# marl/l3embedding

Measured on AMD Instinct MI355X. Metric: AVC training pairs/sec (1s audio + 224x224 frame), higher is better.
Workload: dtype f32; 1 GPU; full cnn_L3_melspec2 AVC training step (audio+vision+fusion, fwd+bwd+Adam), batch 64 per GPU, global batch 64, fp32, inputs resident in HBM; global_batch=64, parallelism=dp1, fp32_conv=f4x4

## Files before the change

include/l3hip.h:

```cpp
#ifndef L3HIP_H
#define L3HIP_H

#include <stdint.h>

#ifdef __cplusplus
extern "C" {
#endif

#define L3_OK 0
#define L3_EINVAL (-1)
#define L3_EHIP (-2)
#define L3_ENOMEM (-3)
#define L3_ESTATE (-4)
#define L3_ECOMM (-5)

#define L3_MODEL_CNN_L3_ORIG 0
#define L3_MODEL_TINY_L3 1
#define L3_MODEL_CNN_L3_KAPREDBINPUTBN 2
#define L3_MODEL_CNN_L3_MELSPEC1 3
#define L3_MODEL_CNN_L3_MELSPEC2 4

typedef struct l3_engine l3_engine;

#define L3_DTYPE_F32 0
// ... 82 lines not shown
int l3_comm_timing(l3_engine *e, int on);
int l3_comm_timing_read(l3_engine *e, double *exposed_ms, double *span_ms, double *bucket_ms, int cap, int *steps);

int l3_grad_arena_dev(l3_engine *e, void **dev_ptr, int64_t *numel);
int l3_bucket_range(const l3_engine *e, int bucket, int64_t *offset, int64_t *numel);
int l3_bn_stats_pack_dev(l3_engine *e, void **send_dev, int64_t *numel);
int l3_bn_stats_replicas_dev(l3_engine *e, int world, void **gathered_dev);

int l3_embed_audio(l3_engine *e, const float *audio, int64_t n, int pool_h, int pool_w, float *out);
int l3_embed_vision(l3_engine *e, const float *video, int64_t n, int pool_h, int pool_w, float *out);
int64_t l3_embed_dim(const l3_engine *e, int vision, int pool_h, int pool_w);
int l3_embed_audio_frames(l3_engine *e, const float *samples, int64_t n_samples, const int64_t *table,
                          int64_t n_frames, int pool_h, int pool_w, float *out);
int l3_embed_audio_clips_resampled(l3_engine *e, const float *native, int64_t n_native, const int64_t *clips,
                                   int64_t n_clips, const double *half_window, int64_t n_window, int num_table,
                                   int64_t n_samples, const int64_t *table, int64_t n_frames, int pool_h, int pool_w,
                                   float *out);

int l3_get_activation(l3_engine *e, const char *name, float *dst, int64_t numel);
int l3_activation_numel(l3_engine *e, const char *name, int64_t *numel);
int l3_sync(l3_engine *e);
int l3_profile_enable(l3_engine *e, int on);
int l3_set_tower_overlap(l3_engine *e, int on);
int l3_profile_read(l3_engine *e, int family, double *ms, int64_t *launches, double *flops);
int l3_profile_read_executed(l3_engine *e, int family, double *flops);
int l3_profile_read_bytes(l3_engine *e, int family, double *bytes);

#define L3_OP_BF16_STORED 2
#define L3_OP_BF16_STORED_OUT 3
int l3_op_conv2d_fwd_dt(int device, int dtype, const float *x, const float *w, const float *b, float *y,
                        int n, int h, int wd, int cin, int cout, int kh, int kw, int same);
int l3_op_conv2d_bwd_dt(int device, int dtype, const float *x, const float *w, const float *dy, float *dx,
                        float *dw, float *db, int n, int h, int wd, int cin, int cout, int kh, int kw, int same);
int l3_op_conv2d_fwd(int device, const float *x, const float *w, const float *b, float *y,
                     int n, int h, int wd, int cin, int cout, int kh, int kw, int same);
int l3_op_conv2d_bwd(int device, const float *x, const float *w, const float *dy,
                     float *dx, float *dw, float *db,
                     int n, int h, int wd, int cin, int cout, int kh, int kw, int same);
int l3_op_bn_relu_fwd(int device, const float *x, const float *gamma, const float *beta,
                      float *y, float *mean, float *var, int64_t rows, int c, int relu, int x_bf16);
int l3_op_bn_relu_bwd(int device, const float *x, const float *y, const float *dy,
                      const float *gamma, const float *beta, const float *mean, const float *var,
                      float *dx, float *dgamma, float *dbeta, int64_t rows, int c, int relu, int x_bf16);
int l3_op_bn_relu_pool2_fwd(int device, const float *x, const float *gamma, const float *beta, float *p,
                            float *mean, float *var, int n, int h, int wd, int c, int same, int relu_mode, int x_bf16);
int l3_op_bn_relu_pool2_bwd(int device, const float *x, const float *gamma, const float *beta, const float *dp,
                            float *dx, float *dgamma, float *dbeta, float *dbias, int n, int h, int wd, int c,
                            int same, int relu_mode, int x_bf16);
int l3_op_maxpool_fwd(int device, const float *x, float *y, int n, int h, int wd, int c,
                      int ph, int pw, int sh, int sw, int same);
int l3_op_maxpool_bwd(int device, const float *x, const float *dy, float *dx, int n, int h,
                      int wd, int c, int ph, int pw, int sh, int sw, int same);
int l3_op_frontend(int device, int model_type, const float *audio, int n, int db_max_scope, float *out);
int l3_op_gather_frames(int device, const float *samples, int64_t n_samples, const int64_t *table,
                        int64_t n_frames, float *frames);
int l3_op_resample(int device, const float *x, int64_t n_in, int64_t sr_orig, int64_t sr_new, const double *half_window,
                   int64_t n_window, int num_table, int64_t t0, int64_t n_out, float *y);
int l3_op_resample_clips(int device, const float *x, int64_t n_in, const int64_t *clips, int64_t n_clips, int64_t sr_new,
                         const double *half_window, int64_t n_window, int num_table, int64_t n_samples, int copy_equal,
                         float *y);
int l3_op_bn_stats_from_partials(int device, const float *part, int nblk, int c, const float *pivot, int64_t rows,
                                 float eps, float *mean, float *var);
int l3_op_preprocess(int device, const uint8_t *video_u8, int64_t nv, float *video,
                     const int16_t *audio_i16, int64_t na, float *audio);
int l3_op_augment_video(int device, const uint8_t *u8, int n, int h, int w, const l3_augment_params *params,
                        uint8_t *out_u8, float *out_f32);
// ... 124 lines not shown
```

l3embedding_amd/_lib.py:

```python
import ctypes as C
import os

import numpy as np

from . import _build

MODEL_IDS = {
    'cnn_L3_orig': 0,
    'tiny_L3': 1,
    'cnn_L3_kapredbinputbn': 2,
    'cnn_L3_melspec1': 3,
    'cnn_L3_melspec2': 4,
}

FAMILIES = ('conv_fwd', 'conv_dgrad', 'conv_wgrad', 'elementwise', 'frontend', 'head', 'adam')


DTYPES = {'f32': 0, 'fp32': 0, 'float32': 0, 'bf16': 1}
FP32_CONV = {'f4x4': 0, 'f2x2': 1, 'f2x2_bf16x6': 2}
DP_MOVING = {'replicas': 0, 'rank_local': 1}
OP_DTYPES = dict(DTYPES, bf16_stored=2, bf16_stored_out=3)


class L3Config(C.Structure):
# ... 60 lines not shown
    'l3_step_results_enqueue': (C.c_int, [C.c_void_p, C.c_int, C.c_int]),
    'l3_step_results_wait': (C.c_int, [C.c_void_p, C.c_int, C.POINTER(C.c_float), C.POINTER(C.c_float)]),
    'l3_comm_unique_id': (C.c_int, [C.c_void_p]),
    'l3_comm_init': (C.c_int, [C.c_void_p, C.c_void_p, C.c_int, C.c_int]),
    'l3_comm_destroy': (C.c_int, [C.c_void_p]),
    'l3_comm_info': (C.c_int, [C.c_void_p, C.POINTER(C.c_int), C.POINTER(C.c_int), C.c_char_p, C.c_int]),
    'l3_comm_allreduce_host': (C.c_int, [C.c_void_p, C.POINTER(C.c_double), C.c_int, C.c_int]),
    'l3_step_dp': (C.c_int, [C.c_void_p, C.c_float]),
    'l3_comm_timing': (C.c_int, [C.c_void_p, C.c_int]),
    'l3_comm_timing_read': (C.c_int, [C.c_void_p, C.POINTER(C.c_double), C.POINTER(C.c_double), C.POINTER(C.c_double), C.c_int, C.POINTER(C.c_int)]),
    'l3_grad_arena_dev': (C.c_int, [C.c_void_p, C.POINTER(C.c_void_p), C.POINTER(C.c_int64)]),
    'l3_bucket_range': (C.c_int, [C.c_void_p, C.c_int, C.POINTER(C.c_int64), C.POINTER(C.c_int64)]),
    'l3_embed_audio': (C.c_int, [C.c_void_p, C.c_void_p, C.c_int64, C.c_int, C.c_int, C.c_void_p]),
    'l3_embed_vision': (C.c_int, [C.c_void_p, C.c_void_p, C.c_int64, C.c_int, C.c_int, C.c_void_p]),
    'l3_embed_dim': (C.c_int64, [C.c_void_p, C.c_int, C.c_int, C.c_int]),
    'l3_embed_audio_frames': (C.c_int, [C.c_void_p, C.c_void_p, C.c_int64, C.c_void_p, C.c_int64, C.c_int, C.c_int,
                                        C.c_void_p]),
    'l3_embed_audio_clips_resampled': (C.c_int, [C.c_void_p, C.c_void_p, C.c_int64, C.c_void_p, C.c_int64, C.c_void_p,
                                                 C.c_int64, C.c_int, C.c_int64, C.c_void_p, C.c_int64, C.c_int, C.c_int,
                                                 C.c_void_p]),
    'l3_get_activation': (C.c_int, [C.c_void_p, C.c_char_p, C.c_void_p, C.c_int64]),
    'l3_activation_numel': (C.c_int, [C.c_void_p, C.c_char_p, C.POINTER(C.c_int64)]),
    'l3_sync': (C.c_int, [C.c_void_p]),
    'l3_profile_enable': (C.c_int, [C.c_void_p, C.c_int]),
    'l3_set_tower_overlap': (C.c_int, [C.c_void_p, C.c_int]),
    'l3_profile_read_executed': (C.c_int, [C.c_void_p, C.c_int, C.POINTER(C.c_double)]),
    'l3_profile_read_bytes': (C.c_int, [C.c_void_p, C.c_int, C.POINTER(C.c_double)]),
    'l3_profile_read': (C.c_int, [C.c_void_p, C.c_int, C.POINTER(C.c_double), C.POINTER(C.c_int64),
                                  C.POINTER(C.c_double)]),
    'l3_op_conv2d_fwd': (C.c_int, [C.c_int, C.c_void_p, C.c_void_p, C.c_void_p, C.c_void_p] + [C.c_int] * 8),
    'l3_op_conv2d_fwd_dt': (C.c_int, [C.c_int, C.c_int, C.c_void_p, C.c_void_p, C.c_void_p, C.c_void_p] + [C.c_int] * 8),
    'l3_op_conv2d_bwd_dt': (C.c_int, [C.c_int, C.c_int] + [C.c_void_p] * 6 + [C.c_int] * 8),
    'l3_op_conv2d_bwd': (C.c_int, [C.c_int] + [C.c_void_p] * 6 + [C.c_int] * 8),
    'l3_op_bn_relu_fwd': (C.c_int, [C.c_int] + [C.c_void_p] * 6 + [C.c_int64, C.c_int, C.c_int, C.c_int]),
    'l3_op_bn_relu_bwd': (C.c_int, [C.c_int] + [C.c_void_p] * 10 + [C.c_int64, C.c_int, C.c_int, C.c_int]),
    'l3_op_bn_relu_pool2_fwd': (C.c_int, [C.c_int] + [C.c_void_p] * 6 + [C.c_int] * 7),
    'l3_op_bn_relu_pool2_bwd': (C.c_int, [C.c_int] + [C.c_void_p] * 8 + [C.c_int] * 7),
    'l3_op_maxpool_fwd': (C.c_int, [C.c_int, C.c_void_p, C.c_void_p] + [C.c_int] * 9),
    'l3_op_maxpool_bwd': (C.c_int, [C.c_int, C.c_void_p, C.c_void_p, C.c_void_p] + [C.c_int] * 9),
    'l3_op_frontend': (C.c_int, [C.c_int, C.c_int, C.c_void_p, C.c_int, C.c_int, C.c_void_p]),
    'l3_op_gather_frames': (C.c_int, [C.c_int, C.c_void_p, C.c_int64, C.c_void_p, C.c_int64, C.c_void_p]),
    'l3_op_resample': (C.c_int, [C.c_int, C.c_void_p, C.c_int64, C.c_int64, C.c_int64, C.c_void_p, C.c_int64, C.c_int,
                                 C.c_int64, C.c_int64, C.c_void_p]),
    'l3_op_resample_clips': (C.c_int, [C.c_int, C.c_void_p, C.c_int64, C.c_void_p, C.c_int64, C.c_int64, C.c_void_p, C.c_int64,
                                       C.c_int, C.c_int64, C.c_int, C.c_void_p]),
    'l3_op_bn_stats_from_partials': (C.c_int, [C.c_int, C.c_void_p, C.c_int, C.c_int, C.c_void_p, C.c_int64, C.c_float,
                                               C.c_void_p, C.c_void_p]),
    'l3_op_preprocess': (C.c_int, [C.c_int, C.c_void_p, C.c_int64, C.c_void_p, C.c_void_p, C.c_int64, C.c_void_p]),
    'l3_op_augment_video': (C.c_int, [C.c_int, C.c_void_p, C.c_int, C.c_int, C.c_int, C.c_void_p, C.c_void_p, C.c_void_p]),
    'l3_op_augment_audio': (C.c_int, [C.c_int, C.c_void_p, C.c_int, C.c_int, C.c_void_p, C.c_void_p, C.c_void_p, C.c_void_p]),
    'l3_mlp_create': (C.c_int, [C.c_int, C.c_int, C.c_int, C.c_int, C.c_float, C.c_uint64, C.POINTER(C.c_void_p)]),
    'l3_mlp_destroy': (None, [C.c_void_p]),
    'l3_mlp_param_count': (C.c_int64, [C.c_void_p]),
    'l3_mlp_set_data': (C.c_int, [C.c_void_p, C.c_void_p, C.c_void_p, C.c_int64, C.c_void_p, C.c_void_p, C.c_int64]),
    'l3_mlp_epoch': (C.c_int, [C.c_void_p, C.c_void_p, C.c_float, C.c_int64, C.POINTER(C.c_double)]),
    'l3_mlp_predict': (C.c_int, [C.c_void_p, C.c_void_p, C.c_int64, C.c_void_p]),
    'l3_mlp_get_weights': (C.c_int, [C.c_void_p, C.c_void_p, C.c_int64]),
    'l3_mlp_set_weights': (C.c_int, [C.c_void_p, C.c_void_p, C.c_int64]),
    'l3_op_mlp_dense_fwd': (C.c_int, [C.c_int, C.c_void_p, C.c_int64, C.c_void_p, C.c_int, C.c_int, C.c_int, C.c_void_p,
                                      C.c_void_p, C.c_int, C.c_void_p]),
    'l3_op_mlp_dense_bwd_x': (C.c_int, [C.c_int, C.c_void_p, C.c_void_p, C.c_void_p, C.c_int, C.c_int, C.c_int, C.c_void_p]),
    'l3_op_mlp_wgrad': (C.c_int, [C.c_int, C.c_void_p, C.c_int64, C.c_void_p, C.c_int, C.c_int, C.c_int, C.c_void_p,
                                  C.c_void_p, C.c_void_p]),
    'l3_op_mlp_wgrad_adam': (C.c_int, [C.c_int, C.c_void_p, C.c_int64, C.c_void_p, C.c_int, C.c_int, C.c_int, C.c_void_p]
                             + [C.c_void_p] * 6 + [C.c_float, C.c_float, C.c_void_p]),
    'l3_op_mlp_softmax_ce': (C.c_int, [C.c_int, C.c_void_p, C.c_void_p, C.c_int, C.c_int, C.c_float] + [C.c_void_p] * 4),
# ... 419 lines not shown

    def profile_enable(self, on=True):
        check(self.lib.l3_profile_enable(self.h, int(on)), self.h)

    def profile_read(self):
        out = {}
        for i, fam in enumerate(FAMILIES):
            ms, n, fl = C.c_double(), C.c_int64(), C.c_double()
            check(self.lib.l3_profile_read(self.h, i, C.byref(ms), C.byref(n), C.byref(fl)), self.h)
            ex = C.c_double()
            check(self.lib.l3_profile_read_executed(self.h, i, C.byref(ex)), self.h)
            by = C.c_double()
            check(self.lib.l3_profile_read_bytes(self.h, i, C.byref(by)), self.h)
            out[fam] = dict(ms=ms.value, launches=n.value, flops=fl.value, executed_flops=ex.value, alg_bytes=by.value)
        return out


def op_conv2d_fwd(x, w, b, same, device=0, dtype='f32'):
    lib = load()
    x, w = _f32(x), _f32(w)
    b = _f32(b)
    n, h, wd, cin = x.shape
    kh, kw, _, cout = w.shape
    ho, wo = (h, wd) if same else (h - kh + 1, wd - kw + 1)
    y = np.empty((n, ho, wo, cout), np.float32)
    if OP_DTYPES[dtype]:
        check(lib.l3_op_conv2d_fwd_dt(device, OP_DTYPES[dtype], _ptr(x), _ptr(w), _ptr(b), _ptr(y), n, h, wd, cin, cout,
                                      kh, kw, int(same)))
    else:
        check(lib.l3_op_conv2d_fwd(device, _ptr(x), _ptr(w), _ptr(b), _ptr(y), n, h, wd, cin, cout, kh, kw, int(same)))
    return y


def op_conv2d_bwd(x, w, dy, same, device=0, dtype='f32'):
    lib = load()
    x, w, dy = _f32(x), _f32(w), _f32(dy)
    n, h, wd, cin = x.shape
    kh, kw, _, cout = w.shape
    dx, dw, db = np.empty_like(x), np.empty_like(w), np.empty((cout,), np.float32)
    if OP_DTYPES[dtype]:
        check(lib.l3_op_conv2d_bwd_dt(device, OP_DTYPES[dtype], _ptr(x), _ptr(w), _ptr(dy), _ptr(dx), _ptr(dw), _ptr(db),
                                      n, h, wd, cin, cout, kh, kw, int(same)))
    else:
        check(lib.l3_op_conv2d_bwd(device, _ptr(x), _ptr(w), _ptr(dy), _ptr(dx), _ptr(dw), _ptr(db),
                                   n, h, wd, cin, cout, kh, kw, int(same)))
    return dx, dw, db


def op_bn_relu_fwd(x, gamma, beta, relu, device=0, x_bf16=False):
    lib = load()
    x = _f32(x)
    c = x.shape[-1]
    rows = x.size // c
    y = np.empty_like(x)
    mean, var = np.empty((c,), np.float32), np.empty((c,), np.float32)
    check(lib.l3_op_bn_relu_fwd(device, _ptr(x), _ptr(_f32(gamma)), _ptr(_f32(beta)), _ptr(y), _ptr(mean),
                                _ptr(var), rows, c, int(relu), int(x_bf16)))
    return y, mean, var


def op_bn_relu_bwd(x, y, dy, gamma, mean, var, relu, device=0, beta=None, x_bf16=False):
    lib = load()
    x, y, dy = _f32(x), _f32(y), _f32(dy)
    c = x.shape[-1]
    rows = x.size // c
    dx = np.empty_like(x)
# ... 737 lines not shown
```

l3embedding_amd/csrc/conv_first.hip:

```cpp
#include "kernels.h"
#include "device_common.h"

#include <stdio.h>
#include <stdlib.h>

namespace l3 {

namespace {

struct FirstArgs {
    const float* x;
    const float* w;
    const float* bias;
    void* y;
    int N, H, W;
    int segs;
    int units;
    int per_wave;
    float* stat_part;
    int stat_mode;
};

constexpr int RUN = 32;

template <int CIN, bool STATS, bool OBF>
__global__ __launch_bounds__(256) void conv_first_fwd_kernel(FirstArgs a) {
    constexpr int ROWF = (RUN + 2) * CIN;
    __shared__ float slab[4][3 * ROWF];
    __shared__ float red[2][4][64];
    const int wave = __builtin_amdgcn_readfirstlane(threadIdx.x >> 6), lane = threadIdx.x & 63;
    float* S = slab[wave];

    float wt[9][CIN];
#pragma unroll
    for (int t9 = 0; t9 < 9; ++t9)
#pragma unroll
        for (int ci = 0; ci < CIN; ++ci) wt[t9][ci] = a.w[(t9 * CIN + ci) * 64 + lane];
    const float bz = a.bias != nullptr ? a.bias[lane] : 0.f;
    const bool srelu = STATS && a.stat_mode == 2;
    const float pivot = srelu ? fmaxf(bz, 0.f) : bz;
    float s0 = 0.f, s1 = 0.f;

    const int gw = blockIdx.x * 4 + wave;
    const int u_begin = gw * a.per_wave;
    const int u_end = min(a.units, u_begin + a.per_wave);
    for (int u = u_begin; u < u_end; ++u) {
        const int seg = u % a.segs, row = u / a.segs;
        const int yy = row % a.H;
        const int x0 = seg * RUN;
#pragma unroll
        for (int r = 0; r < 3; ++r) {
            const int gy = yy - 1 + r;
            const bool rok = (unsigned)gy < (unsigned)a.H;
            const float* src = a.x + ((size_t)(row - 1 + r) * a.W) * CIN;
            for (int f = lane; f < ROWF; f += 64) {
                const int gx = x0 - 1 + f / CIN;
                S[r * ROWF + f] = (rok && (unsigned)gx < (unsigned)a.W) ? src[(size_t)(x0 - 1) * CIN + f] : 0.f;
            }
        }
        __builtin_amdgcn_s_waitcnt(0xc07f);
        __builtin_amdgcn_wave_barrier();
        float win[3][3][CIN];
#pragma unroll
        for (int r = 0; r < 3; ++r)
#pragma unroll
            for (int c = 0; c < 2; ++c)
#pragma unroll
                for (int ci = 0; ci < CIN; ++ci) win[r][c + 1][ci] = S[r * ROWF + c * CIN + ci];
        const size_t out_row = ((size_t)row * a.W + x0) * 64 + lane;
        const int npx = min(RUN, a.W - x0);
#pragma unroll
        for (int px = 0; px < RUN; ++px) {
#pragma unroll
            for (int r = 0; r < 3; ++r)
#pragma unroll
                for (int ci = 0; ci < CIN; ++ci) {
                    win[r][0][ci] = win[r][1][ci];
                    win[r][1][ci] = win[r][2][ci];
                    win[r][2][ci] = S[r * ROWF + (px + 2) * CIN + ci];
                }
            float acc = bz;
#pragma unroll
            for (int r = 0; r < 3; ++r)
#pragma unroll
                for (int c = 0; c < 3; ++c)
#pragma unroll
                    for (int ci = 0; ci < CIN; ++ci) acc = fmaf(win[r][c][ci], wt[r * 3 + c][ci], acc);
            if (px < npx) {
                float yv = acc;
                if constexpr (OBF) {
                    const __bf16 h = (__bf16)acc;
                    reinterpret_cast<__bf16*>(a.y)[out_row + (size_t)px * 64] = h;
                    yv = (float)h;
                } else {
                    __builtin_nontemporal_store(acc, reinterpret_cast<float*>(a.y) + out_row + (size_t)px * 64);
                }
                if constexpr (STATS) {
                    const float d = (srelu ? fmaxf(yv, 0.f) : yv) - pivot;
                    s0 += d;
                    s1 = fmaf(d, d, s1);
                }
            }
        }
        __builtin_amdgcn_wave_barrier();
    }
    if constexpr (STATS) {
        red[0][wave][lane] = s0;
        red[1][wave][lane] = s1;
        __syncthreads();
        if (threadIdx.x < 128) {
            const int which = threadIdx.x >> 6, ch = threadIdx.x & 63;
            a.stat_part[((size_t)blockIdx.x * 2 + which) * 64 + ch] =
                (red[which][0][ch] + red[which][1][ch]) + (red[which][2][ch] + red[which][3][ch]);
        }
    }
}

#ifdef L3_EXPERIMENTS
typedef float f32x2s __attribute__((ext_vector_type(2)));
typedef __bf16 bf16x2s __attribute__((ext_vector_type(2)));
__device__ __forceinline__ void split3_pair(float xa, float xb, unsigned& h1, unsigned& h2, unsigned& h3) {
    h1 = __builtin_bit_cast(unsigned, __builtin_convertvector(f32x2s{xa, xb}, bf16x2s));
    const float ra = xa - __uint_as_float(h1 << 16), rb = xb - __uint_as_float(h1 & 0xffff0000u);
    h2 = __builtin_bit_cast(unsigned, __builtin_convertvector(f32x2s{ra, rb}, bf16x2s));
    const float sa = ra - __uint_as_float(h2 << 16), sb = rb - __uint_as_float(h2 & 0xffff0000u);
    h3 = __builtin_bit_cast(unsigned, __builtin_convertvector(f32x2s{sa, sb}, bf16x2s));
}
__device__ __forceinline__ void split3_oct(const float (&x)[8], bf16x8& t1, bf16x8& t2, bf16x8& t3) {
    unsigned a[4], b[4], c[4];
// ... 168 lines not shown
void launch_first(const FirstArgs& a, int blocks, hipStream_t s, bool out_bf16) {
#ifdef L3_EXPERIMENTS
    const char* x6 = l3_knob("L3_FIRST_FWD_X6");
    if (x6 != nullptr && atoi(x6) != 0) {
        if (a.stat_part != nullptr) {
            if (out_bf16) hipLaunchKernelGGL((conv_first_fwd_x6_kernel<CIN, true, true>), dim3(blocks), dim3(256), 0, s, a);
            else hipLaunchKernelGGL((conv_first_fwd_x6_kernel<CIN, true, false>), dim3(blocks), dim3(256), 0, s, a);
        } else {
            if (out_bf16) hipLaunchKernelGGL((conv_first_fwd_x6_kernel<CIN, false, true>), dim3(blocks), dim3(256), 0, s, a);
            else hipLaunchKernelGGL((conv_first_fwd_x6_kernel<CIN, false, false>), dim3(blocks), dim3(256), 0, s, a);
        }
        return;
    }
#endif
    if (a.stat_part != nullptr) {
        if (out_bf16) hipLaunchKernelGGL((conv_first_fwd_kernel<CIN, true, true>), dim3(blocks), dim3(256), 0, s, a);
        else hipLaunchKernelGGL((conv_first_fwd_kernel<CIN, true, false>), dim3(blocks), dim3(256), 0, s, a);
    } else {
        if (out_bf16) hipLaunchKernelGGL((conv_first_fwd_kernel<CIN, false, true>), dim3(blocks), dim3(256), 0, s, a);
        else hipLaunchKernelGGL((conv_first_fwd_kernel<CIN, false, false>), dim3(blocks), dim3(256), 0, s, a);
    }
}

}

bool conv_first_ok(const ConvGeom& g) {
    const char* env = l3_knob("L3_CONV_FIRST");
    return (env ? atoi(env) : 1) && g.KH == 3 && g.KW == 3 && g.padT == 1 && g.padL == 1 && g.Ho == g.H && g.Wo == g.W &&
           (g.Cin == 1 || g.Cin == 3) && g.Cout == 64 && (size_t)g.N * g.H * ((g.W + RUN - 1) / RUN) < (1ull << 31);
}

int conv_first_stat_blocks(const ConvGeom& g) { return conv_first_ok(g) ? first_blocks(g) : 0; }

void conv_first_fwd(const float* x, const float* w, const float* bias, void* y, const ConvGeom& g, hipStream_t s,
                    float* stat_part, int stat_mode, bool out_bf16) {
    FirstArgs a;
    a.x = x; a.w = w; a.bias = bias; a.y = y;
    a.N = g.N; a.H = g.H; a.W = g.W;
    a.segs = (g.W + RUN - 1) / RUN;
    a.units = g.N * g.H * a.segs;
    const int blocks = first_blocks(g);
    a.per_wave = (a.units + blocks * 4 - 1) / (blocks * 4);
    a.stat_part = stat_part;
    a.stat_mode = stat_mode;
    if (g.Cin == 1)
        launch_first<1>(a, blocks, s, out_bf16);
    else
        launch_first<3>(a, blocks, s, out_bf16);
}

struct FirstWgArgs {
    const float* x;
    const float* dy;
    float* part;
    int N, H, W;
    int segs;
    int units;
    int per_wave;
    FirstWgFuse f;
};

template <int CA, int FUSE, int RELU>
__global__ __launch_bounds__(256) void conv_first_wgrad_kernel(FirstWgArgs a) {
    constexpr int ROWS = 9 * CA, MT = (ROWS + 15) / 16;
    const int lane = threadIdx.x & 63, wave_g = __builtin_amdgcn_readfirstlane(blockIdx.x * 4 + (threadIdx.x >> 6));
    const int l15 = lane & 15, k = lane >> 4;
    int rel[MT], dyy[MT], dxx[MT];
#pragma unroll
    for (int mt = 0; mt < MT; ++mt) {
        const int m = mt * 16 + l15;
        const int tap = m / CA, ci = m - tap * CA;
        const int dh = tap / 3 - 1, dw = tap % 3 - 1;
        rel[mt] = ((dh * a.W + dw) * CA + ci) * 4;
        dyy[mt] = m < ROWS ? dh : -100000;
        dxx[mt] = dw;
    }
    const __amdgpu_buffer_rsrc_t xsrd =
        __builtin_amdgcn_make_buffer_rsrc((void*)a.x, 0, (int)((size_t)a.N * a.H * a.W * CA * 4), 0x00020000);
    constexpr int EB = FUSE == 2 ? 2 : 4;
    const __amdgpu_buffer_rsrc_t ysrd = __builtin_amdgcn_make_buffer_rsrc(
        (void*)(FUSE ? a.f.dA : (const void*)a.dy), 0, (int)((size_t)a.N * a.H * a.W * 64 * EB), 0x00020000);
// ... 142 lines not shown
```

l3embedding_amd/csrc/engine.hip:

```cpp
#include <hip/hip_runtime.h>
#include "knobs.h"

#include <cmath>
#include <cstdio>
#include <cstdlib>
#include <cstring>
#include <map>
#include <string>
#include <vector>

#include "../../include/l3hip.h"
#include "comm.h"
#include "kernels.h"

namespace {

using namespace l3;

static thread_local std::string g_create_error;

constexpr float BN_EPS = 1e-3f;
constexpr float BN_MOMENTUM = 0.99f;
constexpr float L2_WEIGHT = 1e-5f;
constexpr float ADAM_B1 = 0.9f, ADAM_B2 = 0.999f, ADAM_EPS = 1e-8f;
constexpr int AUDIO_T = 48000;

enum ParamKind { PK_KERNEL, PK_BIAS, PK_GAMMA, PK_BETA, PK_MMEAN, PK_MVAR, PK_CONST };
enum OpKind { OP_CONV, OP_BN, OP_RELU, OP_POOL, OP_FLATTEN };
enum Family { F_CONV_FWD, F_CONV_DGRAD, F_CONV_WGRAD, F_ELEMWISE, F_FRONTEND, F_HEAD, F_ADAM, F_COUNT };

struct Tensor {
    float* d = nullptr;
    float* g = nullptr;
    int N = 0, H = 0, W = 0, C = 0;
    int64_t batch_stride = 0;
    bool alias = false;
    bool d_bf16 = false, g_bf16 = false;
    int64_t numel() const { return (int64_t)N * H * W * C; }
    int64_t rows() const { return (int64_t)N * H * W; }
};

struct Param {
    std::string name;
    int ndim = 0;
    int64_t shape[4] = {1, 1, 1, 1};
    bool trainable = false;
    int kind = 0;
    int64_t numel = 0;
    int bucket = 0;
    float* d = nullptr;
    float* g = nullptr;
};

enum ConvFwd { CF_BF16_STORED, CF_BF16_CAST, CF_FIRST, CF_FP32 };
enum ConvWgrad { WG_AUG, WG_AUG_DEFERRED, WG_BF16_STORED, WG_BF16_CAST, WG_FP32 };
enum ConvDgrad { DG_NONE, DG_SMALL, DG_BF16_STORED, DG_BF16_CAST, DG_WINO, DG_FLIPPED };
struct ConvPlan {
    ConvFwd fwd = CF_FP32;
    bool wino_filter = false;
    int stat_mode = 0;
    ConvWgrad wgrad = WG_FP32;
    bool colsum = false;
    ConvDgrad dgrad = DG_NONE;
    int bwd_bn = -1;
    double fwd_executed = -1.0, fwd_bytes = 0.0, wg_executed = -1.0, wg_bytes = 0.0, dg_executed = -1.0, dg_bytes = 0.0;
};
enum BnStats { BS_PARTIALS, BS_FAST, BS_PLAIN, BS_MOVING };
enum BnBwd { BB_BY_FIRST_CONV, BB_FAST_POOLED, BB_FAST, BB_FAST_DEFERRED, BB_PLAIN };
struct BnPlan {
    BnStats stats = BS_MOVING;
    int stat_blocks = 0;
    BnBwd bwd = BB_PLAIN;
    int bwd_blocks = 0;
    double fwd_bytes = 0.0, bwd_bytes = 0.0;
};

struct Op {
    OpKind kind;
    std::string name;
    int in = 0, out = 0;
    int block = 0, bucket = 0;
    int kh = 0, kw = 0, cout = 0;
    bool same = false;
    ConvGeom geom{};
    ConvGeom dgeom{};
    int p_kernel = -1, p_bias = -1;
    float* wflip = nullptr;
    float *wino_uf = nullptr, *wino_ud = nullptr;
    int in_bn = -1;
    bool fused_first = false;
    bool defer_apply = false;
    int bn_defer = -1;
    float *xaug = nullptr, *gaug = nullptr;
    ConvGeom ageom{};
    int bn_follow = -1;
    bool need_dx = true;
    int dy_to_bn = -1;
    float* xwin = nullptr;
    int p_gamma = -1, p_beta = -1, p_mmean = -1, p_mvar = -1;
    bool fused_relu = false;
    bool prerelu = false;
    int fuse_pool = -1;
    int bias_param = -1;
    bool fused_into_bn = false;
// ... 1042 lines not shown
        if ((size_t)blocks * 2 * C <= e->stat_max) return true;
        e->err = cv.name + ": " + std::to_string(blocks) + " partial blocks of " + std::to_string(C) + " channels exceed the statistics scratch (" +
                 std::to_string(e->stat_max) + " floats)";
        return false;
    };
    auto defers = [&](const Op& bn) {
        return training && bn.defer_apply && bn.fuse_pool < 0 && bn_fast_ok(tw.t[bn.in].C) && tw.t[bn.in].d_bf16 == tw.t[bn.out].g_bf16;
    };
    for (auto& op : tw.ops) op.bp = BnPlan{};
    for (auto& op : tw.ops) {
        if (op.kind != OP_CONV) continue;
        op.geom.solo = op.dgeom.solo = solo;
        op.geom.dynamic = op.dgeom.dynamic = e->comm != nullptr ? 1 : 0;
        float* ts = solo ? e->w4_tail : nullptr;
        op.geom.tail_scratch = op.dgeom.tail_scratch = ts;
        op.geom.tail_scratch_bytes = op.dgeom.tail_scratch_bytes = ts ? conv_wino4_tail_scratch_bytes() : 0;

        const Tensor &x = tw.t[op.in], &y = tw.t[op.out];
        const double wbytes = (double)e->params[op.p_kernel].numel * 4.0;
        ConvPlan& p = op.cp = ConvPlan{};
        const bool mp = bf16 && conv_bf16_ok(op.geom);
        p.fwd = mp ? (x.d_bf16 ? CF_BF16_STORED : CF_BF16_CAST) : conv_first_ok(op.geom) ? CF_FIRST : CF_FP32;
        p.wino_filter = op.wino_uf && !mp;
        p.fwd_executed = p.wino_filter ? conv_wino_executed_flops(op.geom) : -1.0;
        p.fwd_bytes = act_bytes(x) + act_bytes(y) + wbytes;
        const int nblk = p.fwd == CF_BF16_STORED ? conv_bf16_stat_blocks(op.geom)
                         : p.fwd == CF_FIRST     ? conv_first_stat_blocks(op.geom)
                         : p.fwd == CF_FP32 && p.wino_filter ? conv_wino_stat_blocks(op.geom) : 0;
        if (epi_stats && training && op.bn_follow >= 0 && e->stat_max > 0 && nblk > 0) {
            if (!fits(op, nblk, op.geom.Cout)) return L3_ESTATE;
            p.stat_mode = tw.ops[op.bn_follow].prerelu ? 2 : 1;
            tw.ops[op.bn_follow].bp.stat_blocks = nblk;
        }
        if (training && op.in_bn >= 0) {
            const Op* fb = op.bn_defer >= 0 && defers(tw.ops[op.bn_defer]) ? &tw.ops[op.bn_defer] : nullptr;
            p.wgrad = fb ? WG_AUG_DEFERRED : WG_AUG;
            p.wg_bytes = (double)x.rows() * op.ageom.Cin * 4.0 + (fb ? act_bytes(tw.t[fb->in]) + grad_bytes(tw.t[fb->out]) : grad_bytes(y));
            continue;
        }
        const bool wbf = bf16 && conv_wgrad_bf16_ok(op.geom);
        p.wgrad = !wbf ? WG_FP32 : x.d_bf16 && y.g_bf16 ? WG_BF16_STORED : WG_BF16_CAST;
        p.wg_executed = conv_wgrad_executed_flops(op.geom, wbf);
        p.wg_bytes = act_bytes(x) + grad_bytes(y) + wbytes;
        p.colsum = !op.bias_by_bn;
        if (!op.need_dx) continue;
        const bool dbf = bf16 && conv_bf16_ok(op.dgeom);
        p.dgrad = conv_dgrad_small_ok(op.geom) ? DG_SMALL
                  : dbf                        ? (y.g_bf16 ? DG_BF16_STORED : DG_BF16_CAST)
                  : op.wino_ud                 ? DG_WINO : DG_FLIPPED;
        p.dg_executed = op.wino_ud && !dbf ? conv_wino_executed_flops(op.dgeom) : -1.0;
        p.dg_bytes = grad_bytes(y) + grad_bytes(x) + wbytes;
        Op* bn = training && op.dy_to_bn >= 0 && e->stat_max > 0 ? &tw.ops[op.dy_to_bn] : nullptr;
        if (bn != nullptr && bn->fuse_pool >= 0 && (bn->xwin == nullptr || x.batch_stride != (int64_t)x.H * x.W * x.C)) bn = nullptr;
        if (bn == nullptr) continue;
        const bool bx = tw.t[bn->in].d_bf16;
        int blocks = -1;
        if (p.dgrad == DG_BF16_STORED && x.g_bf16 && bx && conv_bf16_halo_ok(op.dgeom)) blocks = conv_bf16_stat_blocks(op.dgeom);
        if (p.dgrad == DG_WINO && !x.g_bf16 && !bx && conv_wino_ok(op.dgeom)) blocks = conv_wino_stat_blocks(op.dgeom);
        if (blocks < 0) continue;
        if (!fits(op, blocks, op.dgeom.Cout)) return L3_ESTATE;
        p.bwd_bn = op.dy_to_bn;
        bn->bp.bwd_blocks = blocks;
    }
    for (auto& op : tw.ops) {
        if (op.kind != OP_BN) continue;
        const Tensor &x = tw.t[op.in], &y = tw.t[op.out];
        const Tensor& out = op.fuse_pool >= 0 ? tw.t[tw.ops[op.fuse_pool].out] : y;
        BnPlan& p = op.bp;
        p.stats = !training ? BS_MOVING : p.stat_blocks > 0 ? BS_PARTIALS : op.prerelu || x.d_bf16 ? BS_FAST : BS_PLAIN;
        p.bwd = training && op.fused_first ? BB_BY_FIRST_CONV : !bn_fast_ok(x.C) ? BB_PLAIN : op.fuse_pool >= 0 ? BB_FAST_POOLED
                : defers(op) ? BB_FAST_DEFERRED : BB_FAST;
        p.fwd_bytes = (!training ? 0.0 : p.stat_blocks > 0 ? (double)p.stat_blocks * 2 * x.C * 4 : act_bytes(x)) + act_bytes(x) + act_bytes(out);
        if (p.bwd == BB_BY_FIRST_CONV) p.fwd_bytes += act_bytes(x) + (double)x.rows() * (&op + 1)->ageom.Cin * 4.0;
        if (op.fuse_pool >= 0 && training && op.xwin != nullptr) p.fwd_bytes += (double)out.numel() * (x.d_bf16 ? 2.0 : 4.0);
        p.bwd_bytes = p.bwd == BB_PLAIN ? 2.0 * (act_bytes(x) + grad_bytes(y)) + grad_bytes(x)
                                        : (p.bwd_blocks > 0 ? (double)p.bwd_blocks * 2 * x.C * 4 : act_bytes(x) + grad_bytes(out)) +
                                              (p.bwd == BB_FAST_DEFERRED ? 0.0 : act_bytes(x) + grad_bytes(out) + grad_bytes(x));
    }
    return L3_OK;
}

void tower_forward(l3_engine* e, Tower& tw) {
    const bool training = tw.training;
    for (auto& op : tw.ops) {
        Tensor& x = tw.t[op.in];
        Tensor& y = tw.t[op.out];
        switch (op.kind) {
            case OP_CONV: {
                const ConvPlan& p = op.cp;
                const float *w = e->params[op.p_kernel].d, *bias = e->params[op.p_bias].d;
                float* part = p.stat_mode ? e->stat_scratch : nullptr;
                ProfScope ps(e, F_CONV_FWD, conv_flops(op.geom), op.name.c_str(), p.fwd_executed);
                ps.bytes(p.fwd_bytes);
                if (p.wino_filter) conv_wino_transform_weights(w, op.wino_uf, op.geom, false, e->stream);
                switch (p.fwd) {
                    case CF_BF16_STORED:
                        conv_weights_bf16(w, op.wflip, op.kh, op.kw, x.C, op.cout, true, e->stream);
                        conv_bf16_fwd(x.d, op.wflip, bias, y.d, op.geom, e->stream, true, part, p.stat_mode, y.d_bf16);
                        break;
                    case CF_BF16_CAST:
                        conv_flip_weights(w, op.wflip, op.kh, op.kw, x.C, op.cout, e->stream);
                        conv_bf16_fwd(x.d, op.wflip, bias, y.d, op.geom, e->stream);
                        break;
                    case CF_FIRST:
                        conv_first_fwd(x.d, w, bias, y.d, op.geom, e->stream, part, p.stat_mode, y.d_bf16);
                        break;
                    case CF_FP32:
                        conv_fwd(x.d, w, bias, y.d, op.geom, e->stream, p.wino_filter ? op.wino_uf : nullptr, part, p.stat_mode);
                        break;
                }
                break;
            }
            case OP_BN: {
                const BnPlan& p = op.bp;
                ProfScope ps(e, F_ELEMWISE, 0.0);
                ps.bytes(p.fwd_bytes);
                const float* gamma = e->params[op.p_gamma].d;
                const float* beta = e->params[op.p_beta].d;
                switch (p.stats) {
                    case BS_PARTIALS:
                        bn_stats_from_partials(e->stat_scratch, p.stat_blocks, e->params[op.bias_param].d, gamma, beta, op.mean, op.var,
                                               op.scale, op.shift, x.rows(), x.C, BN_EPS, op.prerelu ? 1 : 0, e->stream);
                        break;
                    case BS_FAST:
                        bn_stats_fast(x.d, gamma, beta, op.mean, op.var, op.scale, op.shift, e->red_scratch, x.rows(), x.C, BN_EPS,
                                      op.prerelu ? 1 : 0, e->stream, x.d_bf16 ? 1 : 0);
                        break;
                    case BS_PLAIN:
                        bn_stats(x.d, gamma, beta, op.mean, op.var, op.scale, op.shift, e->red_scratch, x.rows(), x.C, BN_EPS, e->stream);
                        break;
                    case BS_MOVING:
                        bn_scale_shift(gamma, beta, e->params[op.p_mmean].d, e->params[op.p_mvar].d, op.scale, op.shift, x.C, BN_EPS,
                                       e->stream);
                        break;
                }
                if (p.bwd == BB_BY_FIRST_CONV) bn_xhat_ones(x.d, op.mean, op.var, BN_EPS, (&op + 1)->xaug, x.rows(), x.C, e->stream);
                if (op.fuse_pool >= 0) {
                    Tensor& pl = tw.t[tw.ops[op.fuse_pool].out];
                    bn_relu_pool2_fwd(x.d, op.scale, op.shift, pl.d, x.N, x.H, x.W, x.C, pl.H, pl.W, pl.batch_stride,
                                      op.prerelu ? 2 : (op.fused_relu ? 1 : 0), e->stream, pl.d_bf16 ? 1 : 0, x.d_bf16 ? 1 : 0,
                                      training ? (void*)op.xwin : nullptr);
                } else if (y.d_bf16 || x.d_bf16) {
                    bn_apply_fast(x.d, op.scale, op.shift, y.d, x.rows(), x.C, op.fused_relu ? 1 : 0, e->stream, y.d_bf16 ? 1 : 0,
                                  x.d_bf16 ? 1 : 0);
                } else {
                    bn_apply(x.d, op.scale, op.shift, y.d, x.rows(), x.C, op.fused_relu ? 1 : 0, e->stream);
                }
                break;
            }
            case OP_RELU: {
                if (op.fused_into_bn) break;
                ProfScope ps(e, F_ELEMWISE, 0.0);
                ps.bytes(act_bytes(x) + act_bytes(y));
                relu_fwd(x.d, y.d, x.numel(), e->stream);
                break;
            }
            case OP_POOL: {
                if (op.fused_into_bn) break;
                ProfScope ps(e, F_ELEMWISE, 0.0);
                ps.bytes(act_bytes(x) + act_bytes(y));
                maxpool_fwd(x.d, y.d, op.pg, e->stream);
                break;
            }
            default: break;
        }
    }
}

BnBwdFuse bn_bwd_fuse(const Tower& tw, const Op& bn) {
    return BnBwdFuse{bn.fuse_pool >= 0 ? bn.xwin : tw.t[bn.in].d, bn.scale, bn.shift, bn.mean, bn.var, BN_EPS, bn.fused_relu ? 1 : 0};
}

void tower_backward_block(l3_engine* e, Tower& tw, int block) {
    const bool training = tw.training;
// ... 1483 lines not shown
```

l3embedding_amd/csrc/kernels.h:

```cpp
#pragma once
#include <hip/hip_runtime.h>
#include <stdint.h>

#include <string>
#include <vector>

#include "host_common.h"

namespace l3 {

struct ConvGeom {
    int N, H, W, Cin;
    int Ho, Wo, Cout;
    int KH, KW, padT, padL;
    int f2x2 = 0;
    int solo = 0;
    int dynamic = 0;
    float* tail_scratch = nullptr;
    size_t tail_scratch_bytes = 0;
};
size_t conv_wino4_tail_scratch_bytes();

struct BnBwdFuse {
    const float* x;
// ... 6 lines not shown
              hipStream_t s, const float* wino_u = nullptr, float* bn_part = nullptr, int bn_mode = 0,
              const BnBwdFuse* bn_bwd = nullptr);
bool conv_wino_ok(const ConvGeom& g);
size_t conv_wino_floats(const ConvGeom& g);
double conv_wino_executed_flops(const ConvGeom& g);
void conv_wino_transform_weights(const float* w, float* u, const ConvGeom& g, bool from_fwd_for_dgrad, hipStream_t s);
void conv_wino_fwd(const float* x, const float* u, const float* bias, float* y, const ConvGeom& g, hipStream_t s,
                   float* stat_part = nullptr, int stat_mode = 0, const BnBwdFuse* bn_bwd = nullptr);
int conv_wino_stat_blocks(const ConvGeom& g);
int conv_wino_stat_blocks_max(const ConvGeom& g);
bool conv_dgrad_small_ok(const ConvGeom& g);
bool conv_dgrad_small(const float* dy, const float* w, float* dx, const ConvGeom& g, hipStream_t s);
void conv_flip_weights(const float* w, float* wt, int KH, int KW, int Cin, int Cout, hipStream_t s);
size_t conv_wgrad_scratch_floats(const ConvGeom& g);
bool conv_wgrad_bf16_ok(const ConvGeom& g);
struct FirstWgFuse;
void conv_wgrad(const float* x, const float* dy, float* dw, float* part, const ConvGeom& g,
                hipStream_t s, bool bf16 = false, bool in_bf16 = false, const FirstWgFuse* first_fuse = nullptr);

bool conv_first_ok(const ConvGeom& g);
bool conv_first_wgrad_ok(const ConvGeom& g);
size_t conv_first_wgrad_scratch_floats(const ConvGeom& g);
struct FirstWgFuse {
    const void *bnx, *dA;
    const float *scale, *shift;
    const float *cA, *cB, *cC;
    int relu;
    int bf16;
};
int conv_first_wgrad(const float* x, const float* dy, float* part, const ConvGeom& g, hipStream_t s, const FirstWgFuse* fuse = nullptr);
int conv_first_stat_blocks(const ConvGeom& g);
void conv_first_fwd(const float* x, const float* w, const float* bias, void* y, const ConvGeom& g, hipStream_t s,
                    float* stat_part = nullptr, int stat_mode = 0, bool out_bf16 = false);

bool conv_wgrad_wino_ok(const ConvGeom& g);
int conv_wgrad_wino_splits(const ConvGeom& g, int n);
int conv_wgrad_wino_max_splits(const ConvGeom& g, int n);
double conv_wgrad_wino_executed_flops(const ConvGeom& g);
void conv_wgrad_wino_launch(const float* x, const float* dy, float* part, const ConvGeom& g, int n, hipStream_t s);
void conv_wgrad_wino_finish(const float* part, float* dw, const ConvGeom& g, int splits, hipStream_t s);
double conv_wgrad_executed_flops(const ConvGeom& g, bool bf16);
bool conv_wgrad_bf16_tr_enabled();
void conv_wgrad_bf16_tr_launch(const void* x, const void* dy, float* part, const ConvGeom& g, int n, int splits, hipStream_t s);

bool conv_bf16_ok(const ConvGeom& g);
void conv_bf16_fwd(const float* x, const float* wn, const float* bias, float* y, const ConvGeom& g, hipStream_t s,
                   bool operands_bf16 = false, float* stat_part = nullptr, int stat_mode = 0, bool out_bf16 = false,
                   const BnBwdFuse* bn_bwd = nullptr);
int conv_bf16_stat_blocks(const ConvGeom& g);
bool conv_bf16_halo_ok(const ConvGeom& g);
int conv_bf16_halo_patches(const ConvGeom& g, int n);
void conv_bf16_halo_launch(const void* x, const void* wn, const float* bias, void* y, const ConvGeom& g, int n,
                           hipStream_t s, float* stat_part, int stat_mode, bool out_bf16, const BnBwdFuse* bn_bwd = nullptr);
void conv_weights_bf16(const float* w, void* out, int KH, int KW, int Cin, int Cout, bool flip, hipStream_t s);

void bn_xhat_ones(const float* x, const float* mean, const float* var, float eps, float* xa, int64_t rows, int C,
                  hipStream_t s);
void first_conv_grads(const float* gaug, const float* w, const float* gamma, const float* beta, float* dw, float* dgamma,
                      float* dbeta, float* dbias, int taps, int C, int Co, hipStream_t s);

size_t colreduce_scratch_floats(int64_t rows, int C);
void colsum(const float* x, float* out, float* scratch, int64_t rows, int C, hipStream_t s);
void bn_stats(const float* x, const float* gamma, const float* beta, float* mean, float* var,
              float* scale, float* shift, float* scratch, int64_t rows, int C, float eps,
              hipStream_t s);
void bn_scale_shift(const float* gamma, const float* beta, const float* mean, const float* var,
// ... 151 lines not shown
```

l3embedding_amd/csrc/ops.hip:

```cpp
#include <hip/hip_runtime.h>

#include <cstring>
#include <string>
#include <vector>

#include "../../include/l3hip.h"
#include "kernels.h"
#include "knobs.h"
#include "mlp.h"
#include "vggish.h"

namespace {
using namespace l3;

struct Scope {
    DeviceBufs bufs;
    hipStream_t s = nullptr;
    bool ok = true;
    explicit Scope(int device) : ok(device_ok(device)) {}
    ~Scope() { (void)hipDeviceSynchronize(); }
    template <class T>
    T* alloc(size_t count) {
        T* p = bufs.alloc<T>(count);
        if (!p) ok = false;
// ... 80 lines not shown
    } else if (dtype != L3_DTYPE_F32 && conv_bf16_ok(g)) {
        float* dwn = sc.alloc<float>((size_t)kh * kw * cin * cout);
        if (!sc.ok) return L3_ENOMEM;
        conv_flip_weights(dw, dwn, kh, kw, cin, cout, sc.s);
        conv_bf16_fwd(dx, dwn, db, dy, g, sc.s);
    } else if (conv_first_ok(g)) {
        if (dtype == L3_OP_BF16_STORED_OUT) {
            const size_t ny = (size_t)n * g.Ho * g.Wo * cout;
            uint16_t* yb = sc.alloc<uint16_t>(ny);
            if (!sc.ok) return L3_ENOMEM;
            conv_first_fwd(dx, dw, db, yb, g, sc.s, nullptr, 0, true);
            std::vector<uint16_t> hy(ny);
            sc.get(hy.data(), yb, ny);
            widen_bf16(y, hy.data(), ny);
            return sc.status();
        }
        conv_first_fwd(dx, dw, db, dy, g, sc.s);
    } else {
        float* du = nullptr;
        if (conv_wino_floats(g)) {
            du = sc.alloc<float>(conv_wino_floats(g));
            if (!sc.ok) return L3_ENOMEM;
            conv_wino_transform_weights(dw, du, g, false, sc.s);
        }
        conv_fwd(dx, dw, db, dy, g, sc.s, du);
    }
    sc.get(y, dy, (size_t)n * g.Ho * g.Wo * cout);
    return sc.status();
}

int l3_op_conv2d_fwd(int device, const float* x, const float* w, const float* b, float* y, int n, int h, int wd,
                     int cin, int cout, int kh, int kw, int same) {
    return l3_op_conv2d_fwd_dt(device, L3_DTYPE_F32, x, w, b, y, n, h, wd, cin, cout, kh, kw, same);
}

int l3_op_conv2d_bwd_dt(int device, int dtype, const float* x, const float* w, const float* dy, float* dx, float* dw,
                        float* db, int n, int h, int wd, int cin, int cout, int kh, int kw, int same) {
    Scope sc(device);
    if (!sc.ok) return L3_EHIP;
    const ConvGeom g = make_geom(n, h, wd, cin, cout, kh, kw, same);
    const size_t nx = (size_t)n * h * wd * cin, ny = (size_t)n * g.Ho * g.Wo * cout, nw = (size_t)kh * kw * cin * cout;
    float* d_x = sc.put(x, nx);
    float* d_w = sc.put(w, nw);
    float* d_dy = sc.put(dy, ny);
    float* d_dx = sc.alloc<float>(nx);
    float* d_dw = sc.alloc<float>(nw);
    float* d_db = sc.alloc<float>((size_t)cout);
    float* d_wf = sc.alloc<float>(nw);
    float* d_part = sc.alloc<float>(conv_wgrad_scratch_floats(g));
    float* d_red = sc.alloc<float>(colreduce_scratch_floats((int64_t)n * g.Ho * g.Wo, cout));
    if (!sc.ok) return L3_ENOMEM;
    const bool mp = dtype != L3_DTYPE_F32;
    ConvGeom dg{n, g.Ho, g.Wo, cout, h, wd, cin, kh, kw, kh - 1 - g.padT, kw - 1 - g.padL};
    dg.solo = 1;
    dg.f2x2 = g.f2x2;
    if ((dtype == L3_OP_BF16_STORED || dtype == L3_OP_BF16_STORED_OUT) && conv_wgrad_bf16_ok(g) && conv_bf16_ok(dg)) {
        uint16_t* xb = sc.alloc<uint16_t>(nx);
        uint16_t* gb = sc.alloc<uint16_t>(ny);
        uint16_t* wb = sc.alloc<uint16_t>(2 * nw);
        if (!sc.ok) return L3_ENOMEM;
        cast_bf16(d_x, xb, (int64_t)nx, sc.s);
        cast_bf16(d_dy, gb, (int64_t)ny, sc.s);
        conv_wgrad(reinterpret_cast<const float*>(xb), reinterpret_cast<const float*>(gb), d_dw, d_part, g, sc.s, true, true);
        colsum(d_dy, d_db, d_red, (int64_t)n * g.Ho * g.Wo, cout, sc.s);
        conv_weights_bf16(d_w, wb, kh, kw, cin, cout, false, sc.s);
        if (dtype == L3_OP_BF16_STORED_OUT) {
// ... 867 lines not shown
```

Measured before the change: 2031 pairs/s.

## Recompute first conv inside BN-apply to skip reading its stored output

For the first 3x3 conv (Cin 1 or 3) that is followed by a BN+ReLU, the BN apply step now re-runs the cheap first conv and applies scale/shift/ReLU in-register, so it no longer reads the stored pre-BN activation. An optional mode (knob value 2) drops the raw output store from the first pass, computing only stats, and writes both raw and activated outputs in the recompute pass. The first conv is cheap relative to the memory traffic of a full 64-channel activation, so this trades extra FLOPs for less HBM traffic. Enabled by default in mode 1 (recompute, raw still stored).

```diff
diff --git a/include/l3hip.h b/include/l3hip.h
--- a/include/l3hip.h
+++ b/include/l3hip.h
@@ -138,6 +138,9 @@
                         int n, int h, int wd, int cin, int cout, int kh, int kw, int same);
 int l3_op_conv2d_bwd_dt(int device, int dtype, const float *x, const float *w, const float *dy, float *dx,
                         float *dw, float *db, int n, int h, int wd, int cin, int cout, int kh, int kw, int same);
+int l3_op_conv_first_stat_blocks(int n, int h, int wd, int cin);
+int l3_op_conv_first_bn_relu(int device, int form, const float *x, const float *w, const float *b, const float *scale,
+                             const float *shift, float *y, float *act, float *part, int n, int h, int wd, int cin);
 int l3_op_conv2d_fwd(int device, const float *x, const float *w, const float *b, float *y,
                      int n, int h, int wd, int cin, int cout, int kh, int kw, int same);
 int l3_op_conv2d_bwd(int device, const float *x, const float *w, const float *dy,
diff --git a/l3embedding_amd/_lib.py b/l3embedding_amd/_lib.py
--- a/l3embedding_amd/_lib.py
+++ b/l3embedding_amd/_lib.py
@@ -116,6 +116,8 @@
     'l3_op_conv2d_fwd_dt': (C.c_int, [C.c_int, C.c_int, C.c_void_p, C.c_void_p, C.c_void_p, C.c_void_p] + [C.c_int] * 8),
     'l3_op_conv2d_bwd_dt': (C.c_int, [C.c_int, C.c_int] + [C.c_void_p] * 6 + [C.c_int] * 8),
     'l3_op_conv2d_bwd': (C.c_int, [C.c_int] + [C.c_void_p] * 6 + [C.c_int] * 8),
+    'l3_op_conv_first_stat_blocks': (C.c_int, [C.c_int] * 4),
+    'l3_op_conv_first_bn_relu': (C.c_int, [C.c_int, C.c_int] + [C.c_void_p] * 8 + [C.c_int] * 4),
     'l3_op_bn_relu_fwd': (C.c_int, [C.c_int] + [C.c_void_p] * 6 + [C.c_int64, C.c_int, C.c_int, C.c_int]),
     'l3_op_bn_relu_bwd': (C.c_int, [C.c_int] + [C.c_void_p] * 10 + [C.c_int64, C.c_int, C.c_int, C.c_int]),
     'l3_op_bn_relu_pool2_fwd': (C.c_int, [C.c_int] + [C.c_void_p] * 6 + [C.c_int] * 7),
@@ -601,6 +603,18 @@
     return y
 
 
+def op_conv_first_bn_relu(x, w, b, scale, shift, form, device=0):
+    lib = load()
+    x, w, b, scale, shift = _f32(x), _f32(w), _f32(b), _f32(scale), _f32(shift)
+    n, h, wd, cin = x.shape
+    assert w.shape == (3, 3, cin, 64) and b.shape == scale.shape == shift.shape == (64,)
+    y, act = np.empty((n, h, wd, 64), np.float32), np.empty((n, h, wd, 64), np.float32)
+    part = np.empty((lib.l3_op_conv_first_stat_blocks(n, h, wd, cin), 2, 64), np.float32)
+    check(lib.l3_op_conv_first_bn_relu(device, form, _ptr(x), _ptr(w), _ptr(b), _ptr(scale), _ptr(shift), _ptr(y), _ptr(act),
+                                       _ptr(part), n, h, wd, cin))
+    return y, act, part
+
+
 def op_conv2d_bwd(x, w, dy, same, device=0, dtype='f32'):
     lib = load()
     x, w, dy = _f32(x), _f32(w), _f32(dy)
diff --git a/l3embedding_amd/csrc/conv_first.hip b/l3embedding_amd/csrc/conv_first.hip
--- a/l3embedding_amd/csrc/conv_first.hip
+++ b/l3embedding_amd/csrc/conv_first.hip
@@ -19,12 +19,18 @@
     int per_wave;
     float* stat_part;
     int stat_mode;
+    const float* scale;
+    const float* shift;
+    float* act;
 };
 
 constexpr int RUN = 32;
 
-template <int CIN, bool STATS, bool OBF>
+enum FirstOut { FO_RAW, FO_NONE, FO_ACT, FO_BOTH };
+
+template <int CIN, bool STATS, bool OBF, int OUT = FO_RAW>
 __global__ __launch_bounds__(256) void conv_first_fwd_kernel(FirstArgs a) {
+    static_assert(OUT == FO_RAW || !OBF, "the fused forms store fp32");
     constexpr int ROWF = (RUN + 2) * CIN;
     __shared__ float slab[4][3 * ROWF];
     __shared__ float red[2][4][64];
@@ -40,6 +46,11 @@
     const bool srelu = STATS && a.stat_mode == 2;
     const float pivot = srelu ? fmaxf(bz, 0.f) : bz;
     float s0 = 0.f, s1 = 0.f;
+    float bsc = 0.f, bsh = 0.f;
+    if constexpr (OUT == FO_ACT || OUT == FO_BOTH) {
+        bsc = a.scale[lane];
+        bsh = a.shift[lane];
+    }
 
     const int gw = blockIdx.x * 4 + wave;
     const int u_begin = gw * a.per_wave;
@@ -92,9 +103,11 @@
                     const __bf16 h = (__bf16)acc;
                     reinterpret_cast<__bf16*>(a.y)[out_row + (size_t)px * 64] = h;
                     yv = (float)h;
-                } else {
+                } else if constexpr (OUT == FO_RAW || OUT == FO_BOTH) {
                     __builtin_nontemporal_store(acc, reinterpret_cast<float*>(a.y) + out_row + (size_t)px * 64);
                 }
+                if constexpr (OUT == FO_ACT || OUT == FO_BOTH)
+                    __builtin_nontemporal_store(fmaxf(fmaf(acc, bsc, bsh), 0.f), a.act + out_row + (size_t)px * 64);
                 if constexpr (STATS) {
                     const float d = (srelu ? fmaxf(yv, 0.f) : yv) - pivot;
                     s0 += d;
@@ -329,21 +342,47 @@
 
 int conv_first_stat_blocks(const ConvGeom& g) { return conv_first_ok(g) ? first_blocks(g) : 0; }
 
-void conv_first_fwd(const float* x, const float* w, const float* bias, void* y, const ConvGeom& g, hipStream_t s,
-                    float* stat_part, int stat_mode, bool out_bf16) {
-    FirstArgs a;
+static FirstArgs first_args(const float* x, const float* w, const float* bias, void* y, const ConvGeom& g, int* blocks) {
+    FirstArgs a{};
     a.x = x; a.w = w; a.bias = bias; a.y = y;
     a.N = g.N; a.H = g.H; a.W = g.W;
     a.segs = (g.W + RUN - 1) / RUN;
     a.units = g.N * g.H * a.segs;
-    const int blocks = first_blocks(g);
-    a.per_wave = (a.units + blocks * 4 - 1) / (blocks * 4);
+    *blocks = first_blocks(g);
+    a.per_wave = (a.units + *blocks * 4 - 1) / (*blocks * 4);
+    return a;
+}
+
+void conv_first_fwd(const float* x, const float* w, const float* bias, void* y, const ConvGeom& g, hipStream_t s,
+                    float* stat_part, int stat_mode, bool out_bf16) {
+    int blocks;
+    FirstArgs a = first_args(x, w, bias, y, g, &blocks);
     a.stat_part = stat_part;
     a.stat_mode = stat_mode;
     if (g.Cin == 1)
         launch_first<1>(a, blocks, s, out_bf16);
     else
         launch_first<3>(a, blocks, s, out_bf16);
+}
+
+void conv_first_stats(const float* x, const float* w, const float* bias, const ConvGeom& g, hipStream_t s, float* stat_part,
+                      int stat_mode) {
+    int blocks;
+    FirstArgs a = first_args(x, w, bias, nullptr, g, &blocks);
+    a.stat_part = stat_part;
+    a.stat_mode = stat_mode;
+    auto k = g.Cin == 1 ? conv_first_fwd_kernel<1, true, false, FO_NONE> : conv_first_fwd_kernel<3, true, false, FO_NONE>;
+    hipLaunchKernelGGL(k, dim3(blocks), dim3(256), 0, s, a);
+}
+
+void conv_first_bn_relu(const float* x, const float* w, const float* bias, const float* scale, const float* shift, float* act,
+                        float* y, const ConvGeom& g, hipStream_t s) {
+    int blocks;
+    FirstArgs a = first_args(x, w, bias, y, g, &blocks);
+    a.scale = scale; a.shift = shift; a.act = act;
+    auto k = g.Cin == 1 ? (y != nullptr ? conv_first_fwd_kernel<1, false, false, FO_BOTH> : conv_first_fwd_kernel<1, false, false, FO_ACT>)
+                        : (y != nullptr ? conv_first_fwd_kernel<3, false, false, FO_BOTH> : conv_first_fwd_kernel<3, false, false, FO_ACT>);
+    hipLaunchKernelGGL(k, dim3(blocks), dim3(256), 0, s, a);
 }
 
 struct FirstWgArgs {
diff --git a/l3embedding_amd/csrc/engine.hip b/l3embedding_amd/csrc/engine.hip
--- a/l3embedding_amd/csrc/engine.hip
+++ b/l3embedding_amd/csrc/engine.hip
@@ -52,7 +52,7 @@
     float* g = nullptr;
 };
 
-enum ConvFwd { CF_BF16_STORED, CF_BF16_CAST, CF_FIRST, CF_FP32 };
+enum ConvFwd { CF_BF16_STORED, CF_BF16_CAST, CF_FIRST, CF_FIRST_STATS, CF_FP32 };
 enum ConvWgrad { WG_AUG, WG_AUG_DEFERRED, WG_BF16_STORED, WG_BF16_CAST, WG_FP32 };
 enum ConvDgrad { DG_NONE, DG_SMALL, DG_BF16_STORED, DG_BF16_CAST, DG_WINO, DG_FLIPPED };
 struct ConvPlan {
@@ -66,10 +66,13 @@
     double fwd_executed = -1.0, fwd_bytes = 0.0, wg_executed = -1.0, wg_bytes = 0.0, dg_executed = -1.0, dg_bytes = 0.0;
 };
 enum BnStats { BS_PARTIALS, BS_FAST, BS_PLAIN, BS_MOVING };
+enum BnApply { BA_STORED, BA_FIRST, BA_FIRST_BOTH };
 enum BnBwd { BB_BY_FIRST_CONV, BB_FAST_POOLED, BB_FAST, BB_FAST_DEFERRED, BB_PLAIN };
 struct BnPlan {
     BnStats stats = BS_MOVING;
     int stat_blocks = 0;
+    BnApply apply = BA_STORED;
+    int first_conv = -1;
     BnBwd bwd = BB_PLAIN;
     int bwd_blocks = 0;
     double fwd_bytes = 0.0, bwd_bytes = 0.0;
@@ -1178,6 +1181,17 @@
             p.stat_mode = tw.ops[op.bn_follow].prerelu ? 2 : 1;
             tw.ops[op.bn_follow].bp.stat_blocks = nblk;
         }
+        if (const int ff = knob_int("L3_FIRST_RECOMPUTE", 1); ff != 0 && !bf16 && p.fwd == CF_FIRST && p.stat_mode == 1 && !y.d_bf16) {
+            Op& bn = tw.ops[op.bn_follow];
+            if (bn.in == op.out && bn.fused_relu && bn.fuse_pool < 0 && !tw.t[bn.out].d_bf16) {
+                bn.bp.apply = ff == 2 ? BA_FIRST_BOTH : BA_FIRST;
+                bn.bp.first_conv = (int)(&op - tw.ops.data());
+                if (ff == 2) {
+                    p.fwd = CF_FIRST_STATS;
+                    p.fwd_bytes -= act_bytes(y);
+                }
+            }
+        }
         if (training && op.in_bn >= 0) {
             const Op* fb = op.bn_defer >= 0 && defers(tw.ops[op.bn_defer]) ? &tw.ops[op.bn_defer] : nullptr;
             p.wgrad = fb ? WG_AUG_DEFERRED : WG_AUG;
@@ -1217,6 +1231,10 @@
         p.bwd = training && op.fused_first ? BB_BY_FIRST_CONV : !bn_fast_ok(x.C) ? BB_PLAIN : op.fuse_pool >= 0 ? BB_FAST_POOLED
                 : defers(op) ? BB_FAST_DEFERRED : BB_FAST;
         p.fwd_bytes = (!training ? 0.0 : p.stat_blocks > 0 ? (double)p.stat_blocks * 2 * x.C * 4 : act_bytes(x)) + act_bytes(x) + act_bytes(out);
+        if (p.apply != BA_STORED) {
+            const Op& cv = tw.ops[p.first_conv];
+            p.fwd_bytes += act_bytes(tw.t[cv.in]) + (double)e->params[cv.p_kernel].numel * 4.0 - (p.apply == BA_FIRST ? act_bytes(x) : 0.0);
+        }
         if (p.bwd == BB_BY_FIRST_CONV) p.fwd_bytes += act_bytes(x) + (double)x.rows() * (&op + 1)->ageom.Cin * 4.0;
         if (op.fuse_pool >= 0 && training && op.xwin != nullptr) p.fwd_bytes += (double)out.numel() * (x.d_bf16 ? 2.0 : 4.0);
         p.bwd_bytes = p.bwd == BB_PLAIN ? 2.0 * (act_bytes(x) + grad_bytes(y)) + grad_bytes(x)
@@ -1250,6 +1268,9 @@
                         break;
                     case CF_FIRST:
                         conv_first_fwd(x.d, w, bias, y.d, op.geom, e->stream, part, p.stat_mode, y.d_bf16);
+                        break;
+                    case CF_FIRST_STATS:
+                        conv_first_stats(x.d, w, bias, op.geom, e->stream, part, p.stat_mode);
                         break;
                     case CF_FP32:
                         conv_fwd(x.d, w, bias, y.d, op.geom, e->stream, p.wino_filter ? op.wino_uf : nullptr, part, p.stat_mode);
@@ -1286,6 +1307,10 @@
                     bn_relu_pool2_fwd(x.d, op.scale, op.shift, pl.d, x.N, x.H, x.W, x.C, pl.H, pl.W, pl.batch_stride,
                                       op.prerelu ? 2 : (op.fused_relu ? 1 : 0), e->stream, pl.d_bf16 ? 1 : 0, x.d_bf16 ? 1 : 0,
                                       training ? (void*)op.xwin : nullptr);
+                } else if (p.apply != BA_STORED) {
+                    const Op& cv = tw.ops[p.first_conv];
+                    conv_first_bn_relu(tw.t[cv.in].d, e->params[cv.p_kernel].d, e->params[cv.p_bias].d, op.scale, op.shift, y.d,
+                                       p.apply == BA_FIRST_BOTH ? x.d : nullptr, cv.geom, e->stream);
                 } else if (y.d_bf16 || x.d_bf16) {
                     bn_apply_fast(x.d, op.scale, op.shift, y.d, x.rows(), x.C, op.fused_relu ? 1 : 0, e->stream, y.d_bf16 ? 1 : 0,
                                   x.d_bf16 ? 1 : 0);
diff --git a/l3embedding_amd/csrc/kernels.h b/l3embedding_amd/csrc/kernels.h
--- a/l3embedding_amd/csrc/kernels.h
+++ b/l3embedding_amd/csrc/kernels.h
@@ -62,6 +62,10 @@
 int conv_first_stat_blocks(const ConvGeom& g);
 void conv_first_fwd(const float* x, const float* w, const float* bias, void* y, const ConvGeom& g, hipStream_t s,
                     float* stat_part = nullptr, int stat_mode = 0, bool out_bf16 = false);
+void conv_first_stats(const float* x, const float* w, const float* bias, const ConvGeom& g, hipStream_t s, float* stat_part,
+                      int stat_mode);
+void conv_first_bn_relu(const float* x, const float* w, const float* bias, const float* scale, const float* shift, float* act,
+                        float* y, const ConvGeom& g, hipStream_t s);
 
 bool conv_wgrad_wino_ok(const ConvGeom& g);
 int conv_wgrad_wino_splits(const ConvGeom& g, int n);
diff --git a/l3embedding_amd/csrc/ops.hip b/l3embedding_amd/csrc/ops.hip
--- a/l3embedding_amd/csrc/ops.hip
+++ b/l3embedding_amd/csrc/ops.hip
@@ -136,6 +136,40 @@
 int l3_op_conv2d_fwd(int device, const float* x, const float* w, const float* b, float* y, int n, int h, int wd,
                      int cin, int cout, int kh, int kw, int same) {
     return l3_op_conv2d_fwd_dt(device, L3_DTYPE_F32, x, w, b, y, n, h, wd, cin, cout, kh, kw, same);
+}
+
+int l3_op_conv_first_stat_blocks(int n, int h, int wd, int cin) {
+    const ConvGeom g = make_geom(n, h, wd, cin, 64, 3, 3, 1);
+    return conv_first_stat_blocks(g);
+}
+
+int l3_op_conv_first_bn_relu(int device, int form, const float* x, const float* w, const float* b, const float* scale,
+                             const float* shift, float* y, float* act, float* part, int n, int h, int wd, int cin) {
+    Scope sc(device);
+    if (!sc.ok) return L3_EHIP;
+    const ConvGeom g = make_geom(n, h, wd, cin, 64, 3, 3, 1);
+    if (!conv_first_ok(g) || form < 0 || form > 2) return L3_EINVAL;
+    const size_t ny = (size_t)n * h * wd * 64, np = (size_t)conv_first_stat_blocks(g) * 2 * 64;
+    float* dx = sc.put(x, (size_t)n * h * wd * cin);
+    float* dw = sc.put(w, (size_t)9 * cin * 64);
+    float* db = sc.put(b, 64);
+    float *dsc = sc.put(scale, 64), *dsh = sc.put(shift, 64);
+    float *dy = sc.alloc<float>(ny), *da = sc.alloc<float>(ny), *dp = sc.alloc<float>(np);
+    if (!sc.ok) return L3_ENOMEM;
+    if (form == 0) {
+        conv_first_fwd(dx, dw, db, dy, g, sc.s, dp, 1);
+        bn_apply_fast(dy, dsc, dsh, da, (int64_t)n * h * wd, 64, 1, sc.s);
+    } else {
+        if (form == 1)
+            conv_first_fwd(dx, dw, db, dy, g, sc.s, dp, 1);
+        else
+            conv_first_stats(dx, dw, db, g, sc.s, dp, 1);
+        conv_first_bn_relu(dx, dw, db, dsc, dsh, da, form == 2 ? dy : nullptr, g, sc.s);
+    }
+    sc.get(y, dy, ny);
+    sc.get(act, da, ny);
+    sc.get(part, dp, np);
+    return sc.status();
 }
 
 int l3_op_conv2d_bwd_dt(int device, int dtype, const float* x, const float* w, const float* dy, float* dx, float* dw,
```

Measured after the change: 2030 pairs/s (median of 4 runs). Within noise of the previous version (-0.0%).
